# PhucNguyenAH/tacotron2_subword

Hardware: AMD Instinct MI355X
Metric: mel_frames_per_sec_train (higher is better)
Workload: dtype bf16; 1 GPU; BERT_Tacotron2 default hparams (SMA), full training iteration fwd+loss+bwd+clip+Adam, B=64/GPU, 100 phones, 60 sub-word tokens, 400 frames, 80-mel; global_batch=64, frames_per_item=400, parallelism=dp1, torch_ops=loss reductions, cat/transpose copies, persistent_chains=True, recurrent_steps_bf16=True

## Files before the change

### tacotron2_subword_amd/csrc/gemm.hip

```cpp
#include "kernels.h"
#include <cstdlib>
#include <algorithm>
#include <type_traits>

namespace t2 {

static int g_precision = 0;
static int env_int(const char* name, int dflt) { const char* v = getenv(name); return v && *v ? atoi(v) : dflt; }
static int g_stage = env_int("T2_GEMM_STAGE", 1);
void set_gemm_staging(int on) { g_stage = on != 0; }
static const int g_stage_min = env_int("T2_GEMM_STAGE_MIN", 256);
void set_precision(int p) { g_precision = p; }
int get_precision() { return g_precision; }

namespace {

constexpr int BK = 16;

struct GemmK {
    GemmDesc d;
    int kchunks;
    int avec, bvec;
    int xcd_swizzle;
};
// ... 544 lines not shown
#pragma unroll
    for (int i = 0; i < NB; ++i) {
        const int q = threadIdx.x + i * NT;
        r.b[i] = *reinterpret_cast<const bf16x8*>(B + (long)(q >> 3) * ldb + k0 + (q & 7) * 8);
    }
}
template <bool CONV_A, int NT, int NA, int NB>
__device__ __forceinline__ void finish16(__bf16* __restrict__ as, __bf16* __restrict__ bs, const Raw16<NA, NB>& r) {
#pragma unroll
    for (int i = 0; i < NA; ++i) {
        const int q = threadIdx.x + i * NT;
        bf16x8 a = r.a[i];
        if constexpr (CONV_A) {
            if (!((r.ok >> i) & 1u)) {
#pragma unroll
                for (int j = 0; j < 8; ++j) a[j] = (__bf16)0.f;
            }
        }
        *reinterpret_cast<bf16x8*>(as + swz16(q >> 3, q & 7)) = a;
    }
#pragma unroll
    for (int i = 0; i < NB; ++i) {
        const int q = threadIdx.x + i * NT;
        *reinterpret_cast<bf16x8*>(bs + swz16(q >> 3, q & 7)) = r.b[i];
    }
}

template <bool CONV_A, int WM, int WN, int TM, int TN, int PF>
__global__ __launch_bounds__(64 * WM * WN) void gemm_bf16src_kernel(GemmK g, const __bf16* __restrict__ A16, long lda, const __bf16* __restrict__ B16, long ldb) {
    constexpr int BM = 32 * TM * WM, BN = 32 * TN * WN, NT = 64 * WM * WN, NA = BM * 8 / NT, NB = BN * 8 / NT;
    const ConvAddr cva{g.d.conv_T, g.d.conv_C, g.d.conv_pad};
    int tpos[NA];
    const GemmDesc& d = g.d;
    extern __shared__ __attribute__((aligned(16))) unsigned char smem16[];
    __bf16* const lds = reinterpret_cast<__bf16*>(smem16);
    auto As = [&](int b) { return lds + b * (BM * PK16); };
    auto Bs = [&](int b) { return lds + 2 * (BM * PK16) + b * (BN * PK16); };

    const int split = blockIdx.z;
    int bx = blockIdx.x, by = blockIdx.y;
    if (g.xcd_swizzle) {
        const int gx = gridDim.x, gy = gridDim.y, total = gx * gy;
        const int lin = by * gx + bx;
        const int pid = (lin & 7) * (total >> 3) + (lin >> 3);
        constexpr int GM = 8;
        const int per_group = GM * gx, group = pid / per_group, first_m = group * GM;
        const int gsz = min(gy - first_m, GM);
        by = first_m + (pid % per_group) % gsz;
        bx = (pid % per_group) / gsz;
    }
    const int m0 = by * BM, n0 = bx * BN;
    const int kbeg = split * g.kchunks * BK, kend = min(d.K, kbeg + g.kchunks * BK);
    const __bf16* A = A16 + (long)m0 * lda;
    const __bf16* B = B16 + (long)n0 * ldb;
#pragma unroll
    for (int i = 0; i < NA; ++i) tpos[i] = CONV_A ? (m0 + ((int)(threadIdx.x + i * NT) >> 3)) % cva.T : 0;

    const int lane = threadIdx.x & 63, wave = threadIdx.x >> 6;
    const int wm = wave / WN, wn = wave % WN;
    const int r = lane & 31, h = lane >> 5;

    f32x16 acc[TM][TN];
#pragma unroll
    for (int i = 0; i < TM; ++i)
#pragma unroll
        for (int j = 0; j < TN; ++j)
#pragma unroll
            for (int e = 0; e < 16; ++e) acc[i][j][e] = 0.f;

    auto mma = [&](int buf) {
        const __bf16* as = As(buf);
        const __bf16* bs = Bs(buf);
#pragma unroll
        for (int ks = 0; ks < BK16 / 16; ++ks) {
            bf16x8 a[TM], b[TN];
#pragma unroll
            for (int i = 0; i < TM; ++i) a[i] = *reinterpret_cast<const bf16x8*>(as + swz16(wm * (32 * TM) + i * 32 + r, 2 * ks + h));
#pragma unroll
            for (int j = 0; j < TN; ++j) b[j] = *reinterpret_cast<const bf16x8*>(bs + swz16(wn * (32 * TN) + j * 32 + r, 2 * ks + h));
#pragma unroll
            for (int i = 0; i < TM; ++i)
#pragma unroll
                for (int j = 0; j < TN; ++j) acc[i][j] = __builtin_amdgcn_mfma_f32_32x32x16_bf16(a[i], b[j], acc[i][j], 0, 0, 0);
        }
    };
    const int nks = (kend - kbeg) / BK16;
    if constexpr (PF == 1) {
        if (nks > 0) {
            Raw16<NA, NB> r0;
            issue16<CONV_A, NT>(A, lda, B, ldb, kbeg, cva, tpos, r0);
            finish16<CONV_A, NT>(As(0), Bs(0), r0);
            __syncthreads();
            for (int ks = 0; ks < nks; ++ks) {
                if (ks + 1 < nks) issue16<CONV_A, NT>(A, lda, B, ldb, kbeg + (ks + 1) * BK16, cva, tpos, r0);
                __builtin_amdgcn_sched_barrier(0);
                mma(ks & 1);
                __builtin_amdgcn_sched_barrier(0);
                if (ks + 1 < nks) finish16<CONV_A, NT>(As((ks & 1) ^ 1), Bs((ks & 1) ^ 1), r0);
                __syncthreads();
            }
        }
    } else if (nks > 0) {
        Raw16<NA, NB> r0, r1;
        issue16<CONV_A, NT>(A, lda, B, ldb, kbeg, cva, tpos, r0);
        if (nks > 1) issue16<CONV_A, NT>(A, lda, B, ldb, kbeg + BK16, cva, tpos, r1);
        finish16<CONV_A, NT>(As(0), Bs(0), r0);
        __syncthreads();
        auto step = [&](int ks, Raw16<NA, NB>& nxt, Raw16<NA, NB>& free_) {
            if (ks + 2 < nks) issue16<CONV_A, NT>(A, lda, B, ldb, kbeg + (ks + 2) * BK16, cva, tpos, free_);
            __builtin_amdgcn_sched_barrier(0);
            mma(ks & 1);
            __builtin_amdgcn_sched_barrier(0);
            if (ks + 1 < nks) finish16<CONV_A, NT>(As((ks & 1) ^ 1), Bs((ks & 1) ^ 1), nxt);
            __syncthreads();
        };
        int ks = 0;
        for (; ks + 1 < nks; ks += 2) { step(ks, r1, r0); step(ks + 1, r0, r1); }
        if (ks < nks) step(ks, r1, r0);
    }

    const RngKey key = rng_key(d.seed, d.site);
    float* C = d.C;
    float* ws = d.splitk > 1 ? d.ws + (long)split * (long)d.M * d.N : nullptr;
#pragma unroll
    for (int i = 0; i < TM; ++i)
#pragma unroll
        for (int j = 0; j < TN; ++j) {
            const int n = n0 + wn * (32 * TN) + j * 32 + r;
#pragma unroll
            for (int e = 0; e < 16; ++e) {
                const int m = m0 + wm * (32 * TM) + i * 32 + (e & 3) + 8 * (e >> 2) + 4 * h;
                if (ws) ws[(long)m * d.N + n] = acc[i][j][e];
                else epilogue_store(d, C, m, n, acc[i][j][e], key);
            }
        }
}

template <bool CONV_A, int WM, int WN, int TM, int TN, int PF>
int launch_bf16src(const GemmK& g, const __bf16* pa, long lda, const __bf16* pb, long ldb, int splitk, hipStream_t s) {
    constexpr int BM = 32 * TM * WM, BN = 32 * TN * WN;
    const size_t smem = (size_t)2 * (BM + BN) * PK16 * sizeof(__bf16);
    T2_TRY_RC(t2_allow_dynamic_lds(reinterpret_cast<const void*>(gemm_bf16src_kernel<CONV_A, WM, WN, TM, TN, PF>), smem));
    GemmK gk = g;
    static const int swz = getenv("T2_GEMM_XCD") ? atoi(getenv("T2_GEMM_XCD")) : 1;
    gk.xcd_swizzle = swz && ((g.d.N / BN) * (g.d.M / BM)) % 8 == 0 && (g.d.M / BM) >= 8;
    hipLaunchKernelGGL((gemm_bf16src_kernel<CONV_A, WM, WN, TM, TN, PF>), dim3(g.d.N / BN, g.d.M / BM, splitk), dim3(64 * WM * WN), smem, s, gk, pa, lda, pb, ldb);
    T2_LAUNCH_CHECK();
    return 0;
}

#ifndef T2_G256_PRIO
#define T2_G256_PRIO 1
#endif
template <bool CONV_A>
__global__ __launch_bounds__(512) void gemm_bf16src256_kernel(GemmK g, const __bf16* __restrict__ A16, long lda, const __bf16* __restrict__ B16, long ldb) {
    const GemmDesc& d = g.d;
    extern __shared__ __attribute__((aligned(16))) unsigned char smem16[];
    typedef __attribute__((address_space(3))) void* lds_ptr;
    int bx = blockIdx.x, by = blockIdx.y;
    if (g.xcd_swizzle) {
        const int gx = gridDim.x, gy = gridDim.y, total = gx * gy;
        const int lin = by * gx + bx;
        const int pid = (lin & 7) * (total >> 3) + (lin >> 3);
        constexpr int GM = 4;
        const int per_group = GM * gx, group = pid / per_group, first_m = group * GM;
        const int gsz = min(gy - first_m, GM);
        by = first_m + (pid % per_group) % gsz;
        bx = (pid % per_group) / gsz;
    }
    const int m0 = by * 256, n0 = bx * 256, split = blockIdx.z;
    const int kbeg = split * g.kchunks * BK, kend = min(d.K, kbeg + g.kchunks * BK);
    const int nkt = (kend - kbeg) / 64;
    const int nkt2 = (nkt + 1) & ~1;
    const int tid = threadIdx.x, lane = tid & 63, wave = __builtin_amdgcn_readfirstlane(tid >> 6);
    const int wr = wave >> 2, wc = wave & 3, r = lane & 31, hk = lane >> 5;

    unsigned offA[2][2], offB[2][2];
#pragma unroll
    for (int h = 0; h < 2; ++h)
#pragma unroll
        for (int i = 0; i < 2; ++i) {
            const int s = i * 512 + tid, hr = s >> 3, gc = (s & 7) ^ ((hr >> 1) & 7);
            offA[h][i] = (unsigned)((((hr >> 6) * 128 + h * 64 + (hr & 63)) * lda + gc * 8) * 2);
            offB[h][i] = (unsigned)((((hr >> 5) * 64 + h * 32 + (hr & 31)) * ldb + gc * 8) * 2);
        }
    const ConvAddr cva{d.conv_T, d.conv_C, d.conv_pad};
    int tposA[2][2];
#pragma unroll
    for (int h = 0; h < 2; ++h)
#pragma unroll
        for (int i = 0; i < 2; ++i) {
            const int hr = (i * 512 + tid) >> 3;
            tposA[h][i] = CONV_A ? (m0 + (hr >> 6) * 128 + h * 64 + (hr & 63)) % cva.T : 0;
        }
    int cdk[2], cka[2];
    cdk[0] = cdk[1] = CONV_A ? kbeg / cva.C : 0;
    cka[0] = cka[1] = CONV_A ? kbeg % cva.C : 0;
    auto rsA = CONV_A ? __builtin_amdgcn_make_buffer_rsrc(const_cast<__bf16*>(A16), 0, (int)((long)d.M * lda * 2), 0x00020000)
                      : __builtin_amdgcn_make_buffer_rsrc(const_cast<__bf16*>(A16 + (long)m0 * lda + kbeg), 0, (int)(256 * lda * 2), 0x00020000);
    auto rsB = __builtin_amdgcn_make_buffer_rsrc(const_cast<__bf16*>(B16 + (long)n0 * ldb + kbeg), 0, (int)(256 * ldb * 2), 0x00020000);
    auto stage = [&](int ht, int kt) {
        unsigned char* dst = smem16 + (((kt & 1) * 4 + ht) << 14) + wave * 1024;
        const int ko = kt * 128;
        const bool live = kt < nkt;
        if (ht < 2) {
            if constexpr (CONV_A) {
                const int shift = cdk[ht] - cva.pad;
                const unsigned rel = (unsigned)(((long)(m0 + shift) * lda + cka[ht]) * 2);
                const unsigned o0 = live && (unsigned)(tposA[ht][0] + shift) < (unsigned)cva.T ? offA[ht][0] + rel : 0x80000000u;
                const unsigned o1 = live && (unsigned)(tposA[ht][1] + shift) < (unsigned)cva.T ? offA[ht][1] + rel : 0x80000000u;
                __builtin_amdgcn_raw_ptr_buffer_load_lds(rsA, (lds_ptr)dst, 16, o0, 0, 0, 0);
                __builtin_amdgcn_raw_ptr_buffer_load_lds(rsA, (lds_ptr)(dst + 8192), 16, o1, 0, 0, 0);
                cka[ht] += 64;
                if (cka[ht] == cva.C) { cka[ht] = 0; ++cdk[ht]; }
            } else {
                __builtin_amdgcn_raw_ptr_buffer_load_lds(rsA, (lds_ptr)dst, 16, live ? offA[ht][0] : 0x80000000u, ko, 0, 0);
                __builtin_amdgcn_raw_ptr_buffer_load_lds(rsA, (lds_ptr)(dst + 8192), 16, live ? offA[ht][1] : 0x80000000u, ko, 0, 0);
            }
        } else {
            __builtin_amdgcn_raw_ptr_buffer_load_lds(rsB, (lds_ptr)dst, 16, live ? offB[ht - 2][0] : 0x80000000u, ko, 0, 0);
            __builtin_amdgcn_raw_ptr_buffer_load_lds(rsB, (lds_ptr)(dst + 8192), 16, live ? offB[ht - 2][1] : 0x80000000u, ko, 0, 0);
        }
    };
    const int sw = (r >> 1) & 7;
    unsigned cofs[4];
#pragma unroll
    for (int ks = 0; ks < 4; ++ks) cofs[ks] = (unsigned)(((2 * ks + hk) ^ sw) << 4);
    const unsigned rowA = (unsigned)((wr * 64 + r) * 128), rowB = (unsigned)((wc * 32 + r) * 128);

    f32x16 acc[4][2];
#pragma unroll
    for (int i = 0; i < 4; ++i)
#pragma unroll
        for (int j = 0; j < 2; ++j)
#pragma unroll
            for (int e = 0; e < 16; ++e) acc[i][j][e] = 0.f;
    bf16x8 Af[2][4], Bf[2][4];

    auto read_a = [&](int buf, int h) {
        const unsigned char* base = smem16 + ((buf * 4 + h) << 14) + rowA;
#pragma unroll
        for (int i = 0; i < 2; ++i)
#pragma unroll
            for (int ks = 0; ks < 4; ++ks) Af[i][ks] = *reinterpret_cast<const bf16x8*>(base + i * 4096 + cofs[ks]);
    };
    auto read_b = [&](int buf, int h) {
        const unsigned char* base = smem16 + ((buf * 4 + 2 + h) << 14) + rowB;
#pragma unroll
        for (int ks = 0; ks < 4; ++ks) Bf[h][ks] = *reinterpret_cast<const bf16x8*>(base + cofs[ks]);
    };
    auto mma = [&](int a, int b) {
#if T2_G256_PRIO
        __builtin_amdgcn_s_setprio(1);
#else
        __builtin_amdgcn_sched_barrier(0);
#endif
#pragma unroll
        for (int ks = 0; ks < 4; ++ks)
#pragma unroll
            for (int i = 0; i < 2; ++i) acc[a * 2 + i][b] = __builtin_amdgcn_mfma_f32_32x32x16_bf16(Af[i][ks], Bf[b][ks], acc[a * 2 + i][b], 0, 0, 0);
#if T2_G256_PRIO
        __builtin_amdgcn_s_setprio(0);
#else
        __builtin_amdgcn_sched_barrier(0);
#endif
    };
#define T2_G256_WAIT(N) asm volatile("s_waitcnt vmcnt(" #N ")" ::: "memory")
    auto ktile = [&](auto bufc, auto tailc, int kt) {
        constexpr int BUF = decltype(bufc)::value, TAIL = decltype(tailc)::value;
        read_b(BUF, 0);
        __builtin_amdgcn_sched_barrier(0);
        read_a(BUF, 0);
        if (TAIL < 2) { stage(3, kt + 1); T2_G256_WAIT(8); } else T2_G256_WAIT(2);
        __builtin_amdgcn_s_barrier();
        mma(0, 0);
        __builtin_amdgcn_s_barrier();
        read_b(BUF, 1);
        if (TAIL < 2) { stage(1, kt + 1); T2_G256_WAIT(8); } else T2_G256_WAIT(0);
        __builtin_amdgcn_s_barrier();
        mma(0, 1);
        __builtin_amdgcn_s_barrier();
        read_a(BUF, 1);
        if (TAIL == 0) { stage(0, kt + 2); T2_G256_WAIT(8); }
        __builtin_amdgcn_s_barrier();
        mma(1, 1);
        __builtin_amdgcn_s_barrier();
        if (TAIL == 0) { stage(2, kt + 2); T2_G256_WAIT(8); } else if (TAIL == 1) T2_G256_WAIT(4);
        __builtin_amdgcn_s_barrier();
        mma(1, 0);
        __builtin_amdgcn_s_barrier();
    };
    using I0 = std::integral_constant<int, 0>; using I1 = std::integral_constant<int, 1>; using I2 = std::integral_constant<int, 2>;

    stage(0, 0); stage(2, 0); stage(3, 0); stage(1, 0); stage(0, 1); stage(2, 1);
    T2_G256_WAIT(8);
    __builtin_amdgcn_s_barrier();
    if (wr == 1) __builtin_amdgcn_s_barrier();
    int kt = 0;
    for (; kt + 2 < nkt2; kt += 2) { ktile(I0{}, I0{}, kt); ktile(I1{}, I0{}, kt + 1); }
    ktile(I0{}, I1{}, kt);
    ktile(I1{}, I2{}, kt + 1);
    if (wr == 0) __builtin_amdgcn_s_barrier();
#undef T2_G256_WAIT

    const RngKey key = rng_key(d.seed, d.site);
    float* ws = d.splitk > 1 ? d.ws + (long)split * (long)d.M * d.N : nullptr;
    float* stg = reinterpret_cast<float*>(smem16) + wave * 4096;
    const bool vec_ok = ws || ((reinterpret_cast<uintptr_t>(d.C) & 15) == 0 && d.ldc % 4 == 0);
    const float inv_keep = d.drop_p > 0.f ? 1.0f / (1.0f - d.drop_p) : 1.0f;
    const int c4 = (lane & 15) * 4, n = n0 + wc * 64 + c4;
    f32x4 bias = {0.f, 0.f, 0.f, 0.f};
    if (!ws) {
#pragma unroll
        for (int c = 0; c < 4; ++c) bias[c] = (d.bias1 ? d.bias1[n + c] : 0.f) + (d.bias2 ? d.bias2[n + c] : 0.f);
    }
    __syncthreads();
#pragma unroll
    for (int p = 0; p < 2; ++p) {
#pragma unroll
        for (int ii = 0; ii < 2; ++ii)
#pragma unroll
            for (int j = 0; j < 2; ++j)
#pragma unroll
                for (int e = 0; e < 16; ++e) stg[(ii * 32 + (e & 3) + 8 * (e >> 2) + 4 * hk) * 64 + j * 32 + r] = acc[2 * p + ii][j][e];
        __syncthreads();
        for (int it = 0; it < 16; ++it) {
            const int row = it * 4 + (lane >> 4);
            const int m = m0 + wr * 128 + p * 64 + row;
            f32x4 v = *reinterpret_cast<const f32x4*>(stg + row * 64 + c4);
            if (ws) { *reinterpret_cast<f32x4*>(ws + (long)m * d.N + n) = v; continue; }
            const uint32_t ibase = d.drop_base + (uint32_t)m * d.drop_mstride + (uint32_t)n;
#pragma unroll
            for (int c = 0; c < 4; ++c) {
                float x = apply_act(d.alpha * v[c] + bias[c], d.act);
                if (d.drop_p > 0.f) x = rng_keep(key, ibase + c, d.drop_p) ? x * inv_keep : 0.f;
                v[c] = x;
            }
            const long mo = d.crow_mod ? (long)(m % d.crow_mod) * d.crow_mul + m / d.crow_mod : (long)m;
            float* pc = d.C + mo * d.ldc + n;
            if (vec_ok) {
                if (d.beta != 0.f) v += d.beta * *reinterpret_cast<const f32x4*>(pc);
                *reinterpret_cast<f32x4*>(pc) = v;
            } else {
#pragma unroll
                for (int c = 0; c < 4; ++c) pc[c] = d.beta != 0.f ? v[c] + d.beta * pc[c] : v[c];
            }
        }
        if (p == 0) __syncthreads();
    }
}

template <bool CONV_A>
int launch_bf16src256(const GemmK& g, const __bf16* pa, long lda, const __bf16* pb, long ldb, int splitk, hipStream_t s) {
    constexpr size_t smem = 128 * 1024;
    T2_TRY_RC(t2_allow_dynamic_lds(reinterpret_cast<const void*>(gemm_bf16src256_kernel<CONV_A>), smem));
    GemmK gk = g;
    const int gx = g.d.N / 256, gy = g.d.M / 256;
    gk.xcd_swizzle = (gx * gy) % 8 == 0 && gy >= 4;
    hipLaunchKernelGGL((gemm_bf16src256_kernel<CONV_A>), dim3(gx, gy, splitk), dim3(512), smem, s, gk, pa, lda, pb, ldb);
    T2_LAUNCH_CHECK();
    return 0;
}

__global__ void stage_kc_kernel(const float* __restrict__ src, long ld, __bf16* __restrict__ dst, int rows, int K) {
    const int k8 = K >> 3;
    const long total = (long)rows * k8;
    for (long t = blockIdx.x * (long)blockDim.x + threadIdx.x; t < total; t += (long)gridDim.x * blockDim.x) {
        const long row = t / k8; const int s = (int)(t - row * k8);
        const float* p = src + row * ld + s * 8;
        const f32x4 lo = *reinterpret_cast<const f32x4*>(p), hi = *reinterpret_cast<const f32x4*>(p + 4);
        *reinterpret_cast<bf16x8*>(dst + row * (long)K + s * 8) = pack8(lo, hi);
    }
}
__global__ __launch_bounds__(256) void stage_mc_kernel(const float* __restrict__ src, long ld, __bf16* __restrict__ dst, int rows, int K) {
    __shared__ float tile[64][65];
    const int r0 = blockIdx.x * 64, k0 = blockIdx.y * 64;
#pragma unroll
    for (int i = 0; i < 4; ++i) {
        const int k = (threadIdx.x >> 4) + 16 * i, r4 = (threadIdx.x & 15) * 4;
        const f32x4 v = *reinterpret_cast<const f32x4*>(src + (long)(k0 + k) * ld + r0 + r4);
#pragma unroll
        for (int j = 0; j < 4; ++j) tile[k][r4 + j] = v[j];
    }
    __syncthreads();
#pragma unroll
    for (int i = 0; i < 2; ++i) {
        const int kg = threadIdx.x & 7, row = (threadIdx.x >> 3) + 32 * i;
        bf16x8 o;
#pragma unroll
        for (int j = 0; j < 8; ++j) o[j] = (__bf16)tile[kg * 8 + j][row];
        *reinterpret_cast<bf16x8*>(dst + (long)(r0 + row) * K + k0 + kg * 8) = o;
    }
}

__global__ __launch_bounds__(256) void stage_conv_mc_kernel(const float* __restrict__ X, ConvAddr cv, __bf16* __restrict__ dst, int K) {
    __shared__ float tile[64][65];
    const int r0 = blockIdx.x * 64, k0 = blockIdx.y * 64;
    const int dk = r0 / cv.C, ci0 = r0 - dk * cv.C, shift = dk - cv.pad;
#pragma unroll
    for (int i = 0; i < 4; ++i) {
        const int k = (threadIdx.x >> 4) + 16 * i, r4 = (threadIdx.x & 15) * 4;
        const int m = k0 + k;
        f32x4 v = {0.f, 0.f, 0.f, 0.f};
        if ((unsigned)(m % cv.T + shift) < (unsigned)cv.T) v = *reinterpret_cast<const f32x4*>(X + (long)(m + shift) * cv.C + ci0 + r4);
#pragma unroll
        for (int j = 0; j < 4; ++j) tile[k][r4 + j] = v[j];
    }
    __syncthreads();
#pragma unroll
    for (int i = 0; i < 2; ++i) {
        const int kg = threadIdx.x & 7, row = (threadIdx.x >> 3) + 32 * i;
        bf16x8 o;
#pragma unroll
        for (int j = 0; j < 8; ++j) o[j] = (__bf16)tile[kg * 8 + j][row];
        *reinterpret_cast<bf16x8*>(dst + (long)(r0 + row) * K + k0 + kg * 8) = o;
    }
}

int stage_operand(const float* src, bool kc, long ld, __bf16* dst, int rows, int K, hipStream_t s) {
    if (kc) {
        long blocks = ((long)rows * (K >> 3) + 255) / 256;
        if (blocks > 8192) blocks = 8192;
        hipLaunchKernelGGL(stage_kc_kernel, dim3((unsigned)blocks), dim3(256), 0, s, src, ld, dst, rows, K);
    } else {
        hipLaunchKernelGGL(stage_mc_kernel, dim3(rows / 64, K / 64), dim3(256), 0, s, src, ld, dst, rows, K);
    }
    T2_LAUNCH_CHECK();
    return 0;
}

template <int BM, int BN>
void launch_cfg(const GemmK& g, bool akc, bool bkc, dim3 grid, hipStream_t s) {
    if (akc && bkc) hipLaunchKernelGGL((gemm_kernel<BM, BN, true, true>), grid, dim3(256), 0, s, g);
    else if (akc && !bkc) hipLaunchKernelGGL((gemm_kernel<BM, BN, true, false>), grid, dim3(256), 0, s, g);
    else if (!akc && bkc) hipLaunchKernelGGL((gemm_kernel<BM, BN, false, true>), grid, dim3(256), 0, s, g);
    else hipLaunchKernelGGL((gemm_kernel<BM, BN, false, false>), grid, dim3(256), 0, s, g);
}

inline bool aligned16(const void* p) { return (reinterpret_cast<uintptr_t>(p) & 15) == 0; }

}

int stage_bf16(const float* src, bool kc, long ld, __bf16* dst, int rows, int K, hipStream_t s) {
    T2_REQUIRE(rows > 0 && K > 0 && rows % 64 == 0 && K % 64 == 0 && ld % 4 == 0 && aligned16(src) && aligned16(dst),
               "stage_bf16: rows=%d K=%d ld=%ld must be whole 64-tiles of 16-byte aligned rows", rows, K, ld);
    return stage_operand(src, kc, ld, dst, rows, K, s);
}

int gemm(const GemmDesc& din, hipStream_t s) {
    GemmK g{};
    g.d = din;
    GemmDesc& d = g.d;
    T2_REQUIRE(d.M > 0 && d.N > 0 && d.K > 0 && d.batch > 0, "gemm: bad shape M=%d N=%d K=%d batch=%d", d.M, d.N, d.K, d.batch);
    if (d.conv_a || d.conv_b) {
        T2_REQUIRE(d.conv_T > 0 && d.conv_C > 0 && d.conv_C % 4 == 0 && !(d.conv_a && d.conv_b), "gemm: bad implicit-conv operand (T=%d C=%d)", d.conv_T, d.conv_C);
        T2_REQUIRE(d.batch == 1, "gemm: implicit-conv operands need batch == 1");
        if (d.conv_a) { d.sam = 0; d.sak = 1; T2_REQUIRE(d.K % d.conv_C == 0 && aligned16(d.A), "gemm: conv A operand: K=%d C=%d", d.K, d.conv_C); }
        if (d.conv_b) { d.sbk = 0; d.sbn = 1; T2_REQUIRE(d.N % d.conv_C == 0 && aligned16(d.B), "gemm: conv B operand: N=%d C=%d", d.N, d.conv_C); }
    }
    T2_REQUIRE(d.sam == 1 || d.sak == 1, "gemm: A needs one unit stride (sam=%ld sak=%ld)", d.sam, d.sak);
    T2_REQUIRE(d.sbn == 1 || d.sbk == 1, "gemm: B needs one unit stride (sbn=%ld sbk=%ld)", d.sbn, d.sbk);
    T2_REQUIRE(d.drop_p == 0.f || (d.batch == 1 && (long)d.M * d.N < (1l << 32)), "gemm: dropout epilogue needs batch==1 and M*N < 2^32");
    const bool akc = d.sak == 1, bkc = d.sbk == 1;
    if (d.drop_mstride == 0) d.drop_mstride = (uint32_t)d.N;
    g.avec = aligned16(d.A) && (d.bsA % 4 == 0) && ((akc ? d.sam : d.sak) % 4 == 0);
    g.bvec = aligned16(d.B) && (d.bsB % 4 == 0) && ((bkc ? d.sbn : d.sbk) % 4 == 0);

    const bool use_bf16 = g_precision == 1 && !d.fp32_only && d.M >= 64 && d.N >= 64 && d.K >= 64 &&
                          (!(d.conv_a || d.conv_b) || d.conv_C % 8 == 0);
    bool staged = false;
    __bf16* a16 = nullptr; __bf16* b16 = nullptr;
    const bool conv_any = d.conv_a || d.conv_b;
    if (use_bf16 && g_stage && (!conv_any || (d.conv_C % 64 == 0 && !d.A16 && !d.B16)) && d.batch == 1 && d.M % 128 == 0 && d.N % 128 == 0 && d.K % 64 == 0) {
        const size_t a_elems = d.conv_a ? (size_t)d.M * d.conv_C : (size_t)d.M * d.K;
        const size_t need_a = d.A16 ? 0 : ((a_elems * sizeof(__bf16) + 255) & ~(size_t)255);
        const size_t need_b = d.B16 ? 0 : (((size_t)d.N * d.K * sizeof(__bf16) + 255) & ~(size_t)255);
        const bool big = (d.A16 || d.N >= g_stage_min) && (d.B16 || d.M >= g_stage_min);
        const bool ok_src = (d.A16 || g.avec) && (d.B16 || g.bvec) &&
                            (!d.A16 || (aligned16(d.A16) && d.lda16 % 8 == 0)) && (!d.B16 || (aligned16(d.B16) && d.ldb16 % 8 == 0));
        if (big && ok_src && (need_a + need_b == 0 || (d.ws && aligned16(d.ws) && d.ws_bytes >= need_a + need_b))) {
            staged = true;
            unsigned char* base = reinterpret_cast<unsigned char*>(d.ws);
            if (need_a) a16 = reinterpret_cast<__bf16*>(base);
            if (need_b) b16 = reinterpret_cast<__bf16*>(base + need_a);
            if (need_a + need_b) { d.ws = reinterpret_cast<float*>(base + need_a + need_b); d.ws_bytes -= need_a + need_b; }
        }
    }
    static const int g_t256 = env_int("T2_GEMM_256", 1);
    const bool use256 = staged && g_t256 && d.M % 256 == 0 && d.N % 256 == 0 && d.K >= 128 && (!d.conv_a || (long)d.M * d.conv_C * 2 < (1l << 31));
    int split256 = 1;
    if (use256) {
        const long tiles = (long)(d.M / 256) * (d.N / 256);
        const int nkt = d.K / 64;
        if (d.splitk > 0) split256 = std::min(d.splitk, std::max(1, nkt / 2));
        else if (d.ws && d.beta == 0.f && tiles < 512) {
            double best = 0.0;
            for (int sp = 1; sp <= 16; ++sp) {
                if (sp > 1 && nkt / sp < 16) break;
                const long wgs = tiles * sp, rounds = (wgs + 255) / 256;
                const double eff = (double)wgs / (256.0 * rounds);
                if (eff > best * 1.05) { best = eff; split256 = sp; }
            }
        }
        if (split256 > 1 && !(d.ws && d.beta == 0.f)) split256 = 1;
        if (split256 > 1) {
            const size_t per = (size_t)d.M * d.N * sizeof(float);
            if ((size_t)split256 * per > d.ws_bytes) split256 = (int)(d.ws_bytes / per);
            if (split256 < 1) split256 = 1;
        }
    }
    const int kch = (d.K + BK - 1) / BK;
    const bool can_split = d.ws && d.beta == 0.f && kch >= 64;
    const long tiles128 = (long)((d.M + 127) / 128) * ((d.N + 127) / 128) * d.batch;
    const bool small = !use_bf16 && ((d.M <= 64 || d.N <= 64) || (tiles128 < 256 && !can_split));
    const int BMN = small ? 64 : 128;
    const int tm = (d.M + BMN - 1) / BMN, tn = (d.N + BMN - 1) / BMN;
    int splitk = 1;
    if (d.ws && d.beta == 0.f) {
        splitk = d.splitk;
        if (splitk <= 0) {
            const long tiles = (long)tm * tn * d.batch;
            splitk = 1;
            if (tiles < 512 && kch >= 64) {
                splitk = (int)((1024 + tiles - 1) / tiles);
                if (splitk > kch / 16) splitk = kch / 16;
            }
        }
        const size_t per = (size_t)d.batch * d.M * d.N * sizeof(float);
        if ((size_t)splitk * per > d.ws_bytes) splitk = (int)(d.ws_bytes / per);
        if (splitk < 1) splitk = 1;
    }
    if (use256) splitk = split256;
    g.kchunks = (kch + splitk - 1) / splitk;
    if (use_bf16) g.kchunks = (g.kchunks + 3) & ~3;
    splitk = (kch + g.kchunks - 1) / g.kchunks;
    if (use256 && splitk > 1 && kch - (splitk - 1) * g.kchunks < 8) {
        --splitk;
        g.kchunks = ((kch + splitk - 1) / splitk + 3) & ~3;
        splitk = (kch + g.kchunks - 1) / g.kchunks;
    }
    d.splitk = splitk;
    static const int g_log = env_int("T2_GEMM_LOG", 0);
    if (g_log)
        fprintf(stderr, "t2gemm M=%d N=%d K=%d batch=%d %s%s kernel=%s splitk=%d stageA=%d stageB=%d convA=%d convB=%d beta=%g\n", d.M, d.N, d.K, d.batch,
                akc ? "A[m][k]" : "A[k][m]", bkc ? " B[n][k]" : " B[k][n]", staged ? (use256 ? "src256" : "src128") : use_bf16 ? "bf16conv" : small ? "f32_64" : "f32_128",
                splitk, a16 != nullptr, b16 != nullptr, d.conv_a, d.conv_b, (double)d.beta);
    T2_REQUIRE((long)d.batch * splitk <= 65535, "gemm: batch*splitk too large (%d*%d)", d.batch, splitk);
    dim3 grid(tn, tm, d.batch * splitk);
    if (staged) {
        if (a16) {
            if (d.conv_a) T2_TRY_RC(stage_operand(d.A, true, d.conv_C, a16, d.M, d.conv_C, s));
            else T2_TRY_RC(stage_operand(d.A, akc, akc ? d.sam : d.sak, a16, d.M, d.K, s));
        }
        if (b16) {
            if (d.conv_b) {
                hipLaunchKernelGGL(stage_conv_mc_kernel, dim3(d.N / 64, d.K / 64), dim3(256), 0, s, d.B, ConvAddr{d.conv_T, d.conv_C, d.conv_pad}, b16, d.K);
                T2_LAUNCH_CHECK();
            } else T2_TRY_RC(stage_operand(d.B, bkc, bkc ? d.sbn : d.sbk, b16, d.N, d.K, s));
        }
        const __bf16* pa = d.A16 ? d.A16 : a16; const long lda = d.A16 ? d.lda16 : (d.conv_a ? d.conv_C : d.K);
        const __bf16* pb = d.B16 ? d.B16 : b16; const long ldb = d.B16 ? d.ldb16 : d.K;
        if (use256 && d.conv_a) T2_TRY_RC((launch_bf16src256<true>(g, pa, lda, pb, ldb, splitk, s)));
        else if (use256) T2_TRY_RC((launch_bf16src256<false>(g, pa, lda, pb, ldb, splitk, s)));
        else if (d.conv_a) T2_TRY_RC((launch_bf16src<true, 2, 2, 2, 2, 2>(g, pa, lda, pb, ldb, splitk, s)));
        else T2_TRY_RC((launch_bf16src<false, 2, 2, 2, 2, 2>(g, pa, lda, pb, ldb, splitk, s)));
    } else if (use_bf16) {
        const size_t smem = (size_t)4 * 128 * PK16 * sizeof(__bf16);
        T2_TRY_RC(t2_allow_dynamic_lds(reinterpret_cast<const void*>(gemm_bf16_kernel<true, true>), smem));
        T2_TRY_RC(t2_allow_dynamic_lds(reinterpret_cast<const void*>(gemm_bf16_kernel<true, false>), smem));
        T2_TRY_RC(t2_allow_dynamic_lds(reinterpret_cast<const void*>(gemm_bf16_kernel<false, true>), smem));
        T2_TRY_RC(t2_allow_dynamic_lds(reinterpret_cast<const void*>(gemm_bf16_kernel<false, false>), smem));
        if (akc && bkc) hipLaunchKernelGGL((gemm_bf16_kernel<true, true>), grid, dim3(256), smem, s, g);
        else if (akc && !bkc) hipLaunchKernelGGL((gemm_bf16_kernel<true, false>), grid, dim3(256), smem, s, g);
        else if (!akc && bkc) hipLaunchKernelGGL((gemm_bf16_kernel<false, true>), grid, dim3(256), smem, s, g);
        else hipLaunchKernelGGL((gemm_bf16_kernel<false, false>), grid, dim3(256), smem, s, g);
    } else if (small) launch_cfg<64, 64>(g, akc, bkc, grid, s);
    else launch_cfg<128, 128>(g, akc, bkc, grid, s);
    T2_LAUNCH_CHECK();
    if (splitk > 1) {
        const long total = (long)d.batch * d.M * d.N;
        int blocks = (int)((total + 255) / 256);
        if (blocks > 2048) blocks = 2048;
        hipLaunchKernelGGL(splitk_reduce_kernel, dim3(blocks), dim3(256), 0, s, d);
        T2_LAUNCH_CHECK();
    }
    return 0;
}

}
```

### tacotron2_subword_amd/csrc/kernels.h

```cpp
#pragma once
#include "common.h"

namespace t2 {

enum Act : int { ACT_NONE = 0, ACT_RELU = 1, ACT_TANH = 2 };

struct GemmDesc {
    const float* A; const float* B; float* C;
    int M, N, K;
    long sam, sak;
    long sbn, sbk;
    long ldc;
    int batch; long bsA, bsB, bsC;
    float alpha, beta;
    const float* bias1; const float* bias2;
    int act;
    float drop_p; uint64_t seed; uint32_t site;
    uint32_t drop_base, drop_mstride;
    float* ws; size_t ws_bytes;
    int splitk;
    int conv_a, conv_b, conv_T, conv_C, conv_pad;
    int fp32_only;
    const __bf16* A16; long lda16;
    const __bf16* B16; long ldb16;
    int crow_mod; long crow_mul;
};
inline GemmDesc gemm_desc() {
    GemmDesc d{}; d.batch = 1; d.alpha = 1.f; d.beta = 0.f; d.act = ACT_NONE; d.drop_p = 0.f; return d;
}
int gemm(const GemmDesc& d, hipStream_t s);
int stage_bf16(const float* src, bool kc, long ld, __bf16* dst, int rows, int K, hipStream_t s);
void set_precision(int p);
int get_precision();
void set_gemm_staging(int on);

constexpr int kMaxSeg = 6;
struct LstmSeg { const float* x; long ldx; const float* w; long ldw; int k; };
struct LstmStream {
    LstmSeg seg[kMaxSeg]; int nseg;
    const float* pre; long ldpre;
    const float* bias1; const float* bias2;
    const float* c_prev; long ldc_prev;
    float* gates; long ldgates;
    float* c_new; long ldc_new;
    float* h_out; long ldh_out;
    float* h_out2; long ldh_out2;
    float* c_out; long ldc_out;
    uint32_t site_h, site_c; uint32_t idx_base, idx_bstride;
    const int* lengths; int t;
    const float* wq; int A; float* qpart;
    const __bf16* x16; long ldx16; const __bf16* w16; long ldw16; int k16;
    __bf16* h16_out; long ldh16;
    __bf16* h16_out2; long ldh16_2;
};
constexpr int kMaxLstmStreams = 4;
struct LstmStepDesc { LstmStream st[kMaxLstmStreams]; int nstreams; int B, H; float drop_p; uint64_t seed; };
int lstm_step_fwd(const LstmStepDesc& d, hipStream_t s);

struct LstmBwdStream {
    const float* dh1; long lddh1;
    const float* dh2; long lddh2;
    const float* part; int nparts; long part_stride; long ldpart; int part_col;
    const float* dq; long lddq; const float* wq; int A;
    int dq_parts;
    const float* gates; long ldgates;
    const float* c_new; long ldc_new;
    const float* c_prev; long ldc_prev;
    float* dc_state;
    float* dg; long lddg;
    __bf16* dg16;
    uint32_t site_h, site_c, idx_base, idx_bstride;
};
struct LstmBwdPointDesc { LstmBwdStream st[kMaxLstmStreams]; int nstreams; int B, H; float drop_p; uint64_t seed; int first; };
int lstm_bwd_pointwise(const LstmBwdPointDesc& d, hipStream_t s);

struct LstmBwdSeg { const float* w; long ldw; int ncols; };
struct LstmBwdGemmStream {
    const float* dg; long lddg; LstmBwdSeg seg[3]; int nseg; float* part;
    const __bf16* dg16; const __bf16* wt16;
};
struct LstmBwdGemmDesc { LstmBwdGemmStream st[kMaxLstmStreams]; int nstreams; int B, H4, KS, NC; };
int lstm_bwd_gemm(const LstmBwdGemmDesc& d, hipStream_t s);
int lstm_bwd_ksplit(int H4);
int cast_rows_bf16(const float* src, long ld_src, __bf16* dst, long ld_dst, int R, int C, hipStream_t s);
int cast_transpose_bf16(const float* src, long ld_src, __bf16* dst, long ld_dst, int R, int C, hipStream_t s);

constexpr int kDcaC = 8, kDcaK = 21, kDcaP = 11, kDcaPad = (kDcaK - 1) / 2;
struct DcaWeights {
    const float* bW;
    const float* V;
    const float* F;
    const float* U;
    const float* T; const float* bT;
    const float* v;
    const float* P;
};
struct AttnStream {
    const float* query; long ldq;
    const float* qpart; int nparts;
    float* q_out; long ldq_out;
    const float* pm;
    const float* memory;
    const int* lengths;
    const float* a_prev; long lda_prev;
    float* a_out; long lda_out;
    float* p_out; long ldp_out;
    const float* wcum_prev; long ldwcum_prev;
    float* wcum_out; long ldwcum_out;
    float* ctx1; long ldctx1;
    float* ctx2; long ldctx2;
    __bf16* ctx16; long ldctx16;
    __bf16* ctx16b; long ldctx16b;
    const float* v;
    const float* loc_conv; const float* loc_dense;
    uint32_t site_noise; uint32_t idx_base, idx_bstride;
    int Tin;
    const float* gmm_b1; const float* gmm_w2; const float* gmm_b2;
    const float* mu_prev; float* mu_out;
    DcaWeights dca;
    float mask_value;
};
constexpr int kGmmK = 5, kGmmPad = 8;
struct AttnStepDesc {
    AttnStream st[2]; int nstreams; int B, A, E; int kind;
    int F, Kc; float noise_std; uint64_t seed; int first;
    int lsa_pa;
    int max_pos;
};
int attention_step_fwd(const AttnStepDesc& d, hipStream_t s);

struct AttnBwdStream {
    const float* dctx[3]; long lddctx[3];
    const float* part; int nparts; long part_stride; long ldpart; int part_col;
    const float* dalign; long lddalign;
    const float* q; long ldq;
    const float* pm; const float* memory;
    const float* p; long ldp;
    const float* a_prev; long lda_prev;
    const float* v;
    float* carry;
    float* carry_out;
    float* dctx_out; long lddctx_out;
    float* dq_out; long lddq_out;
    float* dv_acc;
    float* dpm_acc;
    int Tin;
    const float* w; long ldw;
    const float* wcum_prev; long ldwcum_prev;
    const float* loc_conv; const float* loc_dense;
    float* carry_cum;
    float* dconv_acc; float* ddense_acc;
    const float* gmm_w2; const float* gmm_b2;
    const float* mu; long ldmu;
    float* mu_carry;
    float* dw2_acc; float* db2_acc;
    DcaWeights dca;
    float* dca_acc;
};
__host__ __device__ inline size_t dca_acc_floats(int A) { return (size_t)2 * A + 2 * (size_t)A * kDcaC + kDcaC * kDcaK + (size_t)kDcaC * kDcaK * A; }
struct AttnBwdDesc { AttnBwdStream st[2]; int nstreams; int B, A, E; int first; int kind, F, Kc; int nsplit; };
int attention_step_bwd(const AttnBwdDesc& d, hipStream_t s);


enum ChainKind : int { CHAIN_LSTM = 0, CHAIN_SMA = 1, CHAIN_LSA = 2 };
struct ChainStream {
    const __bf16* w16; long ldw16;
    const float* pre;
    const float* wq;
    float* gates; float* c_new; float* c_out;
    float* h_out; long ldh;
    __bf16* h16_out; long ldh16;
    int coff, ctx2off;
    const float* pm; const float* memory; const int* lengths; int Tin;
    float* align; float* psel; float* wcum; float* qs;
    const float* v; const float* loc_conv; const float* loc_dense;
    float* usave; float* locsave;
    uint32_t site_h, site_c, site_noise;
// ... 157 lines not shown
```

Measured before the change: 933,000 mel-frames/s.

## Read k-major operands in 256-tile GEMM via LDS transpose loads

Adds A_T/B_T variants of the 256x256 bf16 GEMM kernel that accept operands stored [k][m]/[k][n]. They load tiles row-contiguous along M/N with a swizzle and use ds_read_tr16_b64 to transpose into MFMA fragments. Staging of fp32 operands that are not k-contiguous now keeps their native layout instead of transposing during the bf16 conversion, so that copy pass reads and writes contiguously. The cost is a more complex kernel with new swizzle and address math and more template instantiations, with a risk of LDS bank conflicts or wrong indexing.

```diff
diff --git a/tacotron2_subword_amd/csrc/gemm.hip b/tacotron2_subword_amd/csrc/gemm.hip
--- a/tacotron2_subword_amd/csrc/gemm.hip
+++ b/tacotron2_subword_amd/csrc/gemm.hip
@@ -720,8 +720,11 @@
 #ifndef T2_G256_PRIO
 #define T2_G256_PRIO 1
 #endif
-template <bool CONV_A>
+typedef __bf16 bf16x4 __attribute__((ext_vector_type(4)));
+__device__ __forceinline__ unsigned tr_swz(int kr) { return (unsigned)(((kr & 3) << 2) | ((kr >> 2) & 3)); }
+template <bool CONV_A, bool A_T, bool B_T>
 __global__ __launch_bounds__(512) void gemm_bf16src256_kernel(GemmK g, const __bf16* __restrict__ A16, long lda, const __bf16* __restrict__ B16, long ldb) {
+    static_assert(!(CONV_A && A_T), "the implicit-im2col A operand is read row-major");
     const GemmDesc& d = g.d;
     extern __shared__ __attribute__((aligned(16))) unsigned char smem16[];
     typedef __attribute__((address_space(3))) void* lds_ptr;
@@ -749,8 +752,11 @@
 #pragma unroll
         for (int i = 0; i < 2; ++i) {
             const int s = i * 512 + tid, hr = s >> 3, gc = (s & 7) ^ ((hr >> 1) & 7);
-            offA[h][i] = (unsigned)((((hr >> 6) * 128 + h * 64 + (hr & 63)) * lda + gc * 8) * 2);
-            offB[h][i] = (unsigned)((((hr >> 5) * 64 + h * 32 + (hr & 31)) * ldb + gc * 8) * 2);
+            const int kr = s >> 4, c = (int)(((unsigned)(s & 15) ^ tr_swz(kr)) * 8);
+            offA[h][i] = A_T ? (unsigned)((kr * lda + (c >> 6) * 128 + h * 64 + (c & 63)) * 2)
+                             : (unsigned)((((hr >> 6) * 128 + h * 64 + (hr & 63)) * lda + gc * 8) * 2);
+            offB[h][i] = B_T ? (unsigned)((kr * ldb + (c >> 5) * 64 + h * 32 + (c & 31)) * 2)
+                             : (unsigned)((((hr >> 5) * 64 + h * 32 + (hr & 31)) * ldb + gc * 8) * 2);
         }
     const ConvAddr cva{d.conv_T, d.conv_C, d.conv_pad};
     int tposA[2][2];
@@ -765,11 +771,14 @@
     cdk[0] = cdk[1] = CONV_A ? kbeg / cva.C : 0;
     cka[0] = cka[1] = CONV_A ? kbeg % cva.C : 0;
     auto rsA = CONV_A ? __builtin_amdgcn_make_buffer_rsrc(const_cast<__bf16*>(A16), 0, (int)((long)d.M * lda * 2), 0x00020000)
+               : A_T  ? __builtin_amdgcn_make_buffer_rsrc(const_cast<__bf16*>(A16 + (long)kbeg * lda + m0), 0, (int)((((long)(kend - kbeg) - 1) * lda + 256) * 2), 0x00020000)
                       : __builtin_amdgcn_make_buffer_rsrc(const_cast<__bf16*>(A16 + (long)m0 * lda + kbeg), 0, (int)(256 * lda * 2), 0x00020000);
-    auto rsB = __builtin_amdgcn_make_buffer_rsrc(const_cast<__bf16*>(B16 + (long)n0 * ldb + kbeg), 0, (int)(256 * ldb * 2), 0x00020000);
+    auto rsB = B_T ? __builtin_amdgcn_make_buffer_rsrc(const_cast<__bf16*>(B16 + (long)kbeg * ldb + n0), 0, (int)((((long)(kend - kbeg) - 1) * ldb + 256) * 2), 0x00020000)
+                   : __builtin_amdgcn_make_buffer_rsrc(const_cast<__bf16*>(B16 + (long)n0 * ldb + kbeg), 0, (int)(256 * ldb * 2), 0x00020000);
+    const int koA = A_T ? (int)(lda * 128) : 128, koB = B_T ? (int)(ldb * 128) : 128;
     auto stage = [&](int ht, int kt) {
         unsigned char* dst = smem16 + (((kt & 1) * 4 + ht) << 14) + wave * 1024;
-        const int ko = kt * 128;
+        const int ko = kt * (ht < 2 ? koA : koB);
         const bool live = kt < nkt;
         if (ht < 2) {
             if constexpr (CONV_A) {
@@ -804,18 +813,49 @@
 #pragma unroll
             for (int e = 0; e < 16; ++e) acc[i][j][e] = 0.f;
     bf16x8 Af[2][4], Bf[2][4];
+    unsigned trA[2][2], trB[2];
+    {
+        const int q = (lane >> 2) & 3, pp = lane & 3, gi = (lane >> 4) & 1;
+#pragma unroll
+        for (int j = 0; j < 2; ++j) {
+            const int kr = 8 * hk + 4 * j + q;
+            const unsigned x = tr_swz(kr), lo = (unsigned)(kr * 256 + 8 * (pp & 1));
+#pragma unroll
+            for (int i = 0; i < 2; ++i) trA[i][j] = lo + ((((unsigned)(wr * 8 + i * 4 + 2 * gi + (pp >> 1))) ^ x) << 4);
+            trB[j] = lo + ((((unsigned)(wc * 4 + 2 * gi + (pp >> 1))) ^ x) << 4);
+        }
+    }
+    typedef __attribute__((address_space(3))) bf16x4* lds_tr_ptr;
+    auto read_tr = [&](const unsigned char* p0, const unsigned char* p1) {
+        const bf16x4 lo = __builtin_amdgcn_ds_read_tr16_b64_v4bf16((lds_tr_ptr)p0), hi = __builtin_amdgcn_ds_read_tr16_b64_v4bf16((lds_tr_ptr)p1);
+        return __builtin_shufflevector(lo, hi, 0, 1, 2, 3, 4, 5, 6, 7);
+    };
 
     auto read_a = [&](int buf, int h) {
-        const unsigned char* base = smem16 + ((buf * 4 + h) << 14) + rowA;
-#pragma unroll
-        for (int i = 0; i < 2; ++i)
-#pragma unroll
-            for (int ks = 0; ks < 4; ++ks) Af[i][ks] = *reinterpret_cast<const bf16x8*>(base + i * 4096 + cofs[ks]);
+        if constexpr (A_T) {
+            const unsigned char* base = smem16 + ((buf * 4 + h) << 14);
+#pragma unroll
+            for (int i = 0; i < 2; ++i)
+#pragma unroll
+                for (int ks = 0; ks < 4; ++ks) Af[i][ks] = read_tr(base + trA[i][0] + ks * 4096, base + trA[i][1] + ks * 4096);
+        } else {
+            const unsigned char* base = smem16 + ((buf * 4 + h) << 14) + rowA;
+#pragma unroll
+            for (int i = 0; i < 2; ++i)
+#pragma unroll
+                for (int ks = 0; ks < 4; ++ks) Af[i][ks] = *reinterpret_cast<const bf16x8*>(base + i * 4096 + cofs[ks]);
+        }
     };
     auto read_b = [&](int buf, int h) {
-        const unsigned char* base = smem16 + ((buf * 4 + 2 + h) << 14) + rowB;
-#pragma unroll
-        for (int ks = 0; ks < 4; ++ks) Bf[h][ks] = *reinterpret_cast<const bf16x8*>(base + cofs[ks]);
+        if constexpr (B_T) {
+            const unsigned char* base = smem16 + ((buf * 4 + 2 + h) << 14);
+#pragma unroll
+            for (int ks = 0; ks < 4; ++ks) Bf[h][ks] = read_tr(base + trB[0] + ks * 4096, base + trB[1] + ks * 4096);
+        } else {
+            const unsigned char* base = smem16 + ((buf * 4 + 2 + h) << 14) + rowB;
+#pragma unroll
+            for (int ks = 0; ks < 4; ++ks) Bf[h][ks] = *reinterpret_cast<const bf16x8*>(base + cofs[ks]);
+        }
     };
     auto mma = [&](int a, int b) {
 #if T2_G256_PRIO
@@ -918,14 +958,14 @@
     }
 }
 
-template <bool CONV_A>
+template <bool CONV_A, bool A_T, bool B_T>
 int launch_bf16src256(const GemmK& g, const __bf16* pa, long lda, const __bf16* pb, long ldb, int splitk, hipStream_t s) {
     constexpr size_t smem = 128 * 1024;
-    T2_TRY_RC(t2_allow_dynamic_lds(reinterpret_cast<const void*>(gemm_bf16src256_kernel<CONV_A>), smem));
+    T2_TRY_RC(t2_allow_dynamic_lds(reinterpret_cast<const void*>(gemm_bf16src256_kernel<CONV_A, A_T, B_T>), smem));
     GemmK gk = g;
     const int gx = g.d.N / 256, gy = g.d.M / 256;
     gk.xcd_swizzle = (gx * gy) % 8 == 0 && gy >= 4;
-    hipLaunchKernelGGL((gemm_bf16src256_kernel<CONV_A>), dim3(gx, gy, splitk), dim3(512), smem, s, gk, pa, lda, pb, ldb);
+    hipLaunchKernelGGL((gemm_bf16src256_kernel<CONV_A, A_T, B_T>), dim3(gx, gy, splitk), dim3(512), smem, s, gk, pa, lda, pb, ldb);
     T2_LAUNCH_CHECK();
     return 0;
 }
@@ -1056,6 +1096,11 @@
     }
     static const int g_t256 = env_int("T2_GEMM_256", 1);
     const bool use256 = staged && g_t256 && d.M % 256 == 0 && d.N % 256 == 0 && d.K >= 128 && (!d.conv_a || (long)d.M * d.conv_C * 2 < (1l << 31));
+    const bool t_ok = use256 && !conv_any;
+    const bool at = d.A16 ? d.a16_t != 0 : (t_ok && !akc && (long)d.K * d.M * 2 < (1l << 31));
+    const bool bt = d.B16 ? d.b16_t != 0 : (t_ok && !bkc && (long)d.K * d.N * 2 < (1l << 31));
+    T2_REQUIRE(!(d.A16 && at) || (t_ok && d.K * d.lda16 * 2 < (1l << 31)), "gemm: A16 stored [k][m] needs the 256-tile kernel (M=%d N=%d K=%d)", d.M, d.N, d.K);
+    T2_REQUIRE(!(d.B16 && bt) || (t_ok && d.K * d.ldb16 * 2 < (1l << 31)), "gemm: B16 stored [k][n] needs the 256-tile kernel (M=%d N=%d K=%d)", d.M, d.N, d.K);
     int split256 = 1;
     if (use256) {
         const long tiles = (long)(d.M / 256) * (d.N / 256);
@@ -1113,23 +1158,31 @@
         fprintf(stderr, "t2gemm M=%d N=%d K=%d batch=%d %s%s kernel=%s splitk=%d stageA=%d stageB=%d convA=%d convB=%d beta=%g\n", d.M, d.N, d.K, d.batch,
                 akc ? "A[m][k]" : "A[k][m]", bkc ? " B[n][k]" : " B[k][n]", staged ? (use256 ? "src256" : "src128") : use_bf16 ? "bf16conv" : small ? "f32_64" : "f32_128",
                 splitk, a16 != nullptr, b16 != nullptr, d.conv_a, d.conv_b, (double)d.beta);
+    if (g_log && (at || bt)) fprintf(stderr, "t2gemm   transposed reads: A16[k][m]=%d B16[k][n]=%d\n", at, bt);
     T2_REQUIRE((long)d.batch * splitk <= 65535, "gemm: batch*splitk too large (%d*%d)", d.batch, splitk);
     dim3 grid(tn, tm, d.batch * splitk);
     if (staged) {
         if (a16) {
             if (d.conv_a) T2_TRY_RC(stage_operand(d.A, true, d.conv_C, a16, d.M, d.conv_C, s));
+            else if (at) T2_TRY_RC(stage_operand(d.A, true, d.sak, a16, d.K, d.M, s));
             else T2_TRY_RC(stage_operand(d.A, akc, akc ? d.sam : d.sak, a16, d.M, d.K, s));
         }
         if (b16) {
             if (d.conv_b) {
                 hipLaunchKernelGGL(stage_conv_mc_kernel, dim3(d.N / 64, d.K / 64), dim3(256), 0, s, d.B, ConvAddr{d.conv_T, d.conv_C, d.conv_pad}, b16, d.K);
                 T2_LAUNCH_CHECK();
-            } else T2_TRY_RC(stage_operand(d.B, bkc, bkc ? d.sbn : d.sbk, b16, d.N, d.K, s));
-        }
-        const __bf16* pa = d.A16 ? d.A16 : a16; const long lda = d.A16 ? d.lda16 : (d.conv_a ? d.conv_C : d.K);
-        const __bf16* pb = d.B16 ? d.B16 : b16; const long ldb = d.B16 ? d.ldb16 : d.K;
-        if (use256 && d.conv_a) T2_TRY_RC((launch_bf16src256<true>(g, pa, lda, pb, ldb, splitk, s)));
-        else if (use256) T2_TRY_RC((launch_bf16src256<false>(g, pa, lda, pb, ldb, splitk, s)));
+            } else if (bt) T2_TRY_RC(stage_operand(d.B, true, d.sbk, b16, d.K, d.N, s));
+            else T2_TRY_RC(stage_operand(d.B, bkc, bkc ? d.sbn : d.sbk, b16, d.N, d.K, s));
+        }
+        const __bf16* pa = d.A16 ? d.A16 : a16; const long lda = d.A16 ? d.lda16 : (d.conv_a ? d.conv_C : at ? d.M : d.K);
+        const __bf16* pb = d.B16 ? d.B16 : b16; const long ldb = d.B16 ? d.ldb16 : (bt ? d.N : d.K);
+        if (use256 && d.conv_a) T2_TRY_RC((launch_bf16src256<true, false, false>(g, pa, lda, pb, ldb, splitk, s)));
+        else if (use256) {
+            if (at && bt) T2_TRY_RC((launch_bf16src256<false, true, true>(g, pa, lda, pb, ldb, splitk, s)));
+            else if (at) T2_TRY_RC((launch_bf16src256<false, true, false>(g, pa, lda, pb, ldb, splitk, s)));
+            else if (bt) T2_TRY_RC((launch_bf16src256<false, false, true>(g, pa, lda, pb, ldb, splitk, s)));
+            else T2_TRY_RC((launch_bf16src256<false, false, false>(g, pa, lda, pb, ldb, splitk, s)));
+        }
         else if (d.conv_a) T2_TRY_RC((launch_bf16src<true, 2, 2, 2, 2, 2>(g, pa, lda, pb, ldb, splitk, s)));
         else T2_TRY_RC((launch_bf16src<false, 2, 2, 2, 2, 2>(g, pa, lda, pb, ldb, splitk, s)));
     } else if (use_bf16) {
diff --git a/tacotron2_subword_amd/csrc/kernels.h b/tacotron2_subword_amd/csrc/kernels.h
--- a/tacotron2_subword_amd/csrc/kernels.h
+++ b/tacotron2_subword_amd/csrc/kernels.h
@@ -23,6 +23,7 @@
     int fp32_only;
     const __bf16* A16; long lda16;
     const __bf16* B16; long ldb16;
+    int a16_t, b16_t;
     int crow_mod; long crow_mul;
 };
 inline GemmDesc gemm_desc() {
```

Result: no change. 933,400 mel-frames/s, median of 5 (+0.0%).
